# CSTR-Edinburgh/magphase

Measured on AMD Instinct MI355X. Metric: frames/sec analysis+synthesis @48kHz FFT=4096, higher is better.
Workload: dtype f32

## Files before the change

include/magphase_hip.h:

```cpp
#ifndef MAGPHASE_HIP_H
#define MAGPHASE_HIP_H

#include <stddef.h>
#include <stdint.h>

#ifdef __cplusplus
extern "C" {
#endif

#define MPX_ABI_VERSION 2

#define MPX_OK 0
#define MPX_ERR_ARG (-1)
#define MPX_ERR_HIP (-2)
#define MPX_ERR_HOST (-3)

int mpx_version(void);
const char* mpx_last_error(void);

size_t mpx_tables_bytes(int fft_len);
int mpx_tables_init(void* stream, int fft_len, void* tables);

int mpx_analysis_frames(void* stream, int fft_len, const void* tables, const float* sig,
                        const int64_t* frame_pos, const int32_t* frame_left, const int32_t* frame_right,
// ... 108 lines not shown
                                   const int32_t* frame_left, const int32_t* frame_right, const int64_t* scratch_off,
                                   int64_t n_frames, float* scratch, int64_t scratch_floats, float* grad_sig,
                                   int64_t total_smpls);

int mpx_analysis_lossless_const_rate_backward(void* stream, int fft_len, const void* tables, const float* mag,
                                              const float* real, const float* imag, int64_t ld, const float* grad_mag,
                                              const float* grad_real, const float* grad_imag, int64_t ld_grad,
                                              int64_t n_const_rows, const int32_t* ranges, const float* row_t,
                                              const int64_t* frame_pos, const int32_t* frame_left,
                                              const int32_t* frame_right, const int64_t* scratch_off, int64_t n_frames,
                                              float* scratch, int64_t scratch_floats, float* grad_sig,
                                              int64_t total_smpls);

int mpx_roundtrip_slot_weights(float* weights_host, int32_t n_slots);
int mpx_roundtrip_frame_terms(int fft_len, const int32_t* frame_left, const int32_t* frame_right, int64_t n_frames,
                              int32_t* terms_host);
int mpx_roundtrip_slot_costs(int32_t* coef_host, int32_t n_slots);
int mpx_roundtrip_lossless_ola(void* stream, int fft_len, const void* tables, const float* sig, const int64_t* frame_pos,
                               const int32_t* frame_left, const int32_t* frame_right, int64_t n_frames,
                               const mpx_ola_run* runs, int32_t n_runs, const int32_t* slot_off, const int32_t* slot_runs,
                               int32_t n_slots, const int32_t* pm_rel, float* out_mag, float* out_real, float* out_imag,
                               float* strips, float* pcm_out, int64_t ld);
#define MPX_RT_FULL_SUPPORT 1u
#define MPX_RT_STORE_ROWS 4u
#define MPX_RT_STORE_NT 8u
#define MPX_RT_INVERSE_TRANSFORM 32u
int mpx_roundtrip_store_map(int fft_len, int phase, int32_t* out);
int mpx_roundtrip_lossless_ola_flags(void* stream, int fft_len, const void* tables, const float* sig,
                                     const int64_t* frame_pos, const int32_t* frame_left, const int32_t* frame_right,
                                     int64_t n_frames, const mpx_ola_run* runs, int32_t n_runs, const int32_t* slot_off,
                                     const int32_t* slot_runs, int32_t n_slots, const int32_t* pm_rel, float* out_mag,
                                     float* out_real, float* out_imag, float* strips, float* pcm_out, int64_t ld,
                                     uint32_t flags);
int mpx_roundtrip_support_classes(int fft_len, const int32_t* frame_left, const int32_t* frame_right, int64_t n_frames,
                                  int32_t* class_host);
int mpx_roundtrip_frame_extents(int fft_len, const int32_t* frame_left, const int32_t* frame_right, int64_t n_frames,
                                uint32_t flags, int32_t* extents_host);

int mpx_griffin_lim_ola(void* stream, int fft_len, const void* tables, const float* sig_in, const int64_t* frame_pos,
                        const int32_t* frame_left, const int32_t* frame_right, int64_t n_frames, const float* target_mag,
                        const mpx_ola_run* runs, int32_t n_runs, const int32_t* slot_off, const int32_t* slot_runs,
                        int32_t n_slots, const int32_t* pm_rel, float* phase_out, float* strips, float* sig_out,
                        int64_t ld);

#define MPX_GL_FOLD_HALF 0
#define MPX_GL_FOLD_FULL 1
#define MPX_GL_FOLD_WORDS 2
int mpx_griffin_lim_fold(void* stream, int fft_len, int32_t form, const float* mag, const void* phase, int64_t ld_phase,
                         int64_t frame0, int64_t n_frames, float* out_mag, float* out_real, float* out_imag,
                         float* out_phase, int64_t ld);


int mpx_mel_unwarp(void* stream, int64_t n_frames, int32_t n_bins, const float* a_mag, int32_t k_mag,
                   const float* u_mag, float* out_mag, const float* a_real, const float* a_imag, int32_t k_phase,
                   const float* u_phase, float* out_real, float* out_imag,
                   int64_t ld );

int mpx_mel_unwarp_rows(void* stream, int64_t n_frames, int32_t n_bins, const float* a_mag, int32_t k_mag,
                        const float* u_mag, float* out_mag, const float* a_real, const float* a_imag, int32_t k_phase,
                        const float* u_phase, float* out_real, float* out_imag, int64_t ld, const int32_t* row0,
                        const int32_t* row1, const float* row_t, int64_t n_rows, const int32_t* tile_first,
                        const int32_t* voiced, int32_t n_phase_bins);

int64_t mpx_spec_ld(int32_t n_bins);

int mpx_noise_uniform(void* stream, int32_t n_utts, const uint64_t* seeds, const int64_t* offsets, int64_t max_len,
// ... 282 lines not shown
```

magphase_amd/_lib.py:

```python
import ctypes
import threading
import os

_HERE = os.path.dirname(os.path.abspath(__file__))
LIB_PATH = os.path.join(_HERE, "libmagphase_hip.so")

vp, i32, i64, sz, f64 = ctypes.c_void_p, ctypes.c_int32, ctypes.c_int64, ctypes.c_size_t, ctypes.c_double
u32 = ctypes.c_uint32

PROTOTYPES = {
    "mpx_version": (i32, []),
    "mpx_last_error": (ctypes.c_char_p, []),
    "mpx_tables_bytes": (sz, [i32]),
    "mpx_tables_init": (i32, [vp, i32, vp]),
    "mpx_feat_ld": (i64, [i32]),
    "mpx_analysis_frames": (i32, [vp, i32] + [vp] * 5 + [i64, vp, vp, vp, i64]),
    "mpx_tables_f64_bytes": (sz, [i32]),
    "mpx_tables_f64_init": (i32, [vp, i32, vp]),
    "mpx_analysis_frames_f64": (i32, [vp, i32] + [vp] * 5 + [i64, vp, vp, vp, i64, vp]),
    "mpx_analysis_frames_f64w": (i32, [vp, i32] + [vp] * 5 + [i64, vp, vp, vp, i64, vp, vp, i32]),
    "mpx_analysis_compressed_fused": (i32, [vp, i32] + [vp] * 5 + [i64, vp, i32, vp, vp, i32, i32, vp, i32, vp, vp,
                                       vp]),
    "mpx_analysis_compressed_fused_cr": (i32, [vp, i32] + [vp] * 5 + [i64, vp, i32, vp, vp, i32, i32] + [vp] * 4 +
                                          [i64] + [vp] * 4),
    "mpx_analysis_compressed_fused_cr_work_bytes": (i64, [i32, i64]),
    "mpx_analysis_compressed_fused_tiles": (i32, [i32, i32, ctypes.POINTER(i32), ctypes.POINTER(i32)]),
    "mpx_analysis_compressed_fused_waves": (i32, []),
    "mpx_analysis_compressed_fused_layout": (i32, []),
    "mpx_analysis_compressed_fused_blocks_per_cu": (i32, [i32, i32]),
    "mpx_synthesis_lossless_frames": (i32, [vp, i32] + [vp] * 4 + [i64, vp, i64]),
    "mpx_ola_gather": (i32, [vp, i32, vp, i32] + [vp] * 4 + [i64, vp]),
    "mpx_synth_ola_slots": (i32, []),
    "mpx_synth_ola_slot_weights": (i32, [vp, i32]),
    "mpx_ola_strip_floats": (i64, [i32]),
    "mpx_synthesis_lossless_ola": (i32, [vp, i32] + [vp] * 5 + [i32, vp, vp, i32, vp, vp, vp, i64]),
    "mpx_synthesis_lossless_ola_lerp": (i32, [vp, i32] + [vp] * 8 + [i32, vp, vp, i32, vp, vp, vp, i64]),
    "mpx_rows_lerp": (i32, [vp, i32, vp, vp, vp, i64, vp, vp, vp, i64, vp, vp, vp, i64]),
    "mpx_synthesis_lossless_backward": (i32, [vp, i32, vp, vp, i64, vp, vp, vp, i64, vp, vp, vp, i64] + [vp] * 6 + [i64]),
    "mpx_synthesis_compressed_backward": (i32, [vp, i32, vp, vp, i64, vp, vp, vp, i64, vp, vp, vp, i64] + [vp] * 12
                                          + [i32, vp, vp, vp, i64]),
    "mpx_synthesis_compressed_type2_backward": (i32, [vp, i32, vp, vp, i64, vp, vp, vp, i64, vp, vp, vp, i64] + [vp] * 12
                                                + [i32, vp, vp, vp, i64]),
    "mpx_rows_lerp_adjoint": (i32, [vp, i32, vp, vp, vp, i64, vp, vp, i64, vp, vp, vp, i64]),
    "mpx_analysis_lossless_backward": (i32, [vp, i32, vp, vp, vp, vp, i64, vp, vp, vp, i64, vp, vp, vp, vp, i64, vp, i64,
                                             vp, i64]),
    "mpx_analysis_lossless_const_rate_backward": (i32, [vp, i32, vp, vp, vp, vp, i64, vp, vp, vp, i64, i64, vp, vp, vp, vp,
                                                        vp, vp, i64, vp, i64, vp, i64]),
    "mpx_ola_fixup": (i32, [vp, i32, vp, i32, vp, vp]),
    "mpx_ola_fixup_width": (i32, [vp, i32, vp, i32, vp, vp, i32]),
    "mpx_roundtrip_lossless_ola": (i32, [vp, i32] + [vp] * 5 + [i64, vp, i32, vp, vp, i32] + [vp] * 6 + [i64]),
    "mpx_roundtrip_lossless_ola_flags": (i32, [vp, i32] + [vp] * 5 + [i64, vp, i32, vp, vp, i32] + [vp] * 6 + [i64, u32]),
    "mpx_roundtrip_support_classes": (i32, [i32, vp, vp, i64, vp]),
    "mpx_roundtrip_frame_extents": (i32, [i32, vp, vp, i64, u32, vp]),
    "mpx_roundtrip_store_map": (i32, [i32, i32, vp]),
    "mpx_roundtrip_slot_weights": (i32, [vp, i32]),
    "mpx_roundtrip_frame_terms": (i32, [i32, vp, vp, i64, vp]),
    "mpx_roundtrip_slot_costs": (i32, [vp, i32]),
    "mpx_griffin_lim_ola": (i32, [vp, i32] + [vp] * 5 + [i64, vp, vp, i32, vp, vp, i32] + [vp] * 4 + [i64]),
    "mpx_griffin_lim_fold": (i32, [vp, i32, i32, vp, vp, i64, i64, i64, vp, vp, vp, vp, i64]),
    "mpx_mel_unwarp": (i32, [vp, i64, i32, vp, i32] + [vp] * 4 + [i32, vp, vp, vp, i64]),
    "mpx_mel_unwarp_rows": (i32, [vp, i64, i32, vp, i32] + [vp] * 4 + [i32, vp, vp, vp, i64, vp, vp, vp, i64, vp, vp,
                             i32]),
    "mpx_spec_ld": (i64, [i32]),
    "mpx_noise_uniform": (i32, [vp, i32, vp, vp, i64, vp]),
    "mpx_noise_numpy_mt19937": (i32, [vp, vp, i32, i64] + [vp] * 5),
    "mpx_noise_numpy_mt19937_work_words": (i64, []),
    "mpx_host_mt19937_jump_poly": (i32, [i64, i32, vp]),
    "mpx_host_mt19937_jump_polys": (i32, [vp, i32, vp, i32]),
    "mpx_noise_stats": (i32, [vp, i32] + [vp] * 6 + [i64, vp]),
    "mpx_noise_spectra_floats": (i64, [i32, i64]),
    "mpx_noise_stats_spectra": (i32, [vp, i32] + [vp] * 6 + [i64, vp, vp]),
    "mpx_synth_comp_slots": (i32, []),
    "mpx_synth_comp_slot_weights": (i32, [vp, i32]),
    "mpx_synthesis_compressed_ola": (i32, [vp, i32] + [vp] * 21 + [i32, vp, vp, i32, vp, vp, i64, i32]),
    "mpx_synthesis_compressed_type2_ola": (i32, [vp, i32] + [vp] * 21 + [i32, vp, vp, i32, vp, vp, i64, i32]),
    "mpx_synthesis_compressed_ola_spectra": (i32, [vp, i32] + [vp] * 21 + [i32, vp, vp, i32, vp, vp, i64, i32, vp]),
    "mpx_host_const_to_var_scan": (i64, [vp, vp, i64, vp, vp]),
    "mpx_host_const_to_var_scan_cap": (i64, [vp, vp, i64, vp, vp, i64]),
    "mpx_host_plan_analysis": (i64, [i32] + [vp] * 12),
    "mpx_host_plan_analysis_batch": (i64, [i32] + [vp] * 8 + [i32] + [vp] * 9 + [i32, vp, vp, i64, vp, i32]),
    "mpx_host_plan_synthesis": (i64, [i32, vp, vp, f64, i32, i32, i32, i64] + [vp] * 17),
    "mpx_host_plan_synthesis_batch": (i64, [i32] + [vp] * 5 + [i32, i32, vp, vp, f64] + [i32] * 4 + [vp, f64, i32, vp,
                                       i64] + [vp] * 9 + [i64, vp, i32]),
    "mpx_host_plan_lossless_synthesis": (i64, [i32, vp, vp, vp, i32] + [vp] * 4),
# ... 25 lines not shown
    "mpx_post_filter": (i32, [vp, vp, i64, i32, vp, i32, i32, vp, vp]),
    "mpx_epoch_f0_track": (i32, [vp, vp, vp, i32, i32, vp, i64, vp, vp, vp, i64] + [i32] * 4 + [f64, vp, vp, vp]),
    "mpx_epoch_zff": (i32, [vp, vp, vp, i32, i64, vp, i32, vp, vp, vp, i32] + [vp] * 5),
    "mpx_pcm16": (i32, [vp, vp, i32, vp, i32, i64, f64, vp, vp]),
    "mpx_pcm16_to_f32": (i32, [vp, vp, i64, vp]),
    "mpx_hpf_block": (i32, []),
    "mpx_output_hpf": (i32, [vp] * 4 + [i32, i64] + [vp] * 7),
    "mpx_bw_probe": (i32, [vp, i32, vp, vp, i64]),
    "mpx_bw_probe_shapes": (i32, []),
    "mpx_rows_pack": (i32, [vp, vp, vp, i32, i32] + [vp, i32, i64, i64] * 3),
    "mpx_post_filter_merlin": (i32, [vp, vp, i64, i32] + [vp] * 4 + [i32, f64, vp, f64] + [vp] * 5),
    "mpx_post_filter_backward": (i32, [vp, vp, i64, i32, vp, vp, vp, i32, vp]),
    "mpx_post_filter_merlin_backward": (i32, [vp, vp, vp, i64, i32] + [vp] * 4 + [i32] + [vp] * 7),
    "mpx_mlpg_work_doubles": (i64, [i64, i32]),
    "mpx_mlpg_solve": (i32, [vp, vp, i32, i64, vp, i32, i64, vp, i32, i64, i32, i32, vp, i32, vp, i64, vp]),
    "mpx_mlpg_apply": (i32, [vp, vp, i32, i64, vp, i32, i64, vp, i32, i64, i32, i32, vp, vp, i64]),
    "mpx_mlpg_colsum_work_doubles": (i64, [i64, i64]),
    "mpx_mlpg_column_sums": (i32, [vp, vp, i64, i64, i64, vp, vp]),
    "mpx_mlpg_var_backward": (i32, [vp, vp, i64, vp, i64, vp, i32, i64, vp, i32, i64, vp, i32, i64, i32, i32, vp, vp, i64,
                                    vp, vp]),
    "mpx_mlpg_trajectory_nll": (i32, [vp, vp, i64, vp, i32, i64, vp, i32, i64, vp, i32, i64, i32, i32, vp, vp]),
    "mpx_mlpg_nll_work_doubles": (i64, [i64, i32]),
    "mpx_mlpg_trajectory_nll_backward": (i32, [vp, vp, i32, i64, vp, i32, i64, vp, i64, vp, i32, i64, vp, vp, i32, i64,
                                               i32, i32, vp, vp, i64, vp, i64, vp]),
    "mpx_cmp_voiced_neighbours": (i32, [vp, vp, i32, i64, vp, i32, i64, vp]),
    "mpx_cmp_compose": (i32, [vp, vp, i32, i64, vp, i32, i32, i32, f64, i32, vp, vp, i32, i64, i32, vp, vp, vp, vp, i32,
                              i64]),
    "mpx_cmp_compose_backward": (i32, [vp, vp, i64, vp, i32, i32, i32, vp, vp, i32, i64, i32, vp, vp, vp, i64]),
    "mpx_cmp_moments_work_doubles": (i64, [i64, i64]),
    "mpx_cmp_column_moments": (i32, [vp, vp, i32, i64, i64, i64, vp, vp]),
}
SYMBOLS = tuple(PROTOTYPES)
RT_STORE_FLAGS = {"rows": 4, "lines": 0, "lines_nt": 8}
RT_INVERSE_FLAGS = {"direct": 0, "transform": 32}
del vp, i32, i64, sz, f64

_lib = None


class MagphaseHipError(RuntimeError):
    pass


_load_lock = threading.Lock()


def load():
    global _lib
    if _lib is not None:
        return _lib
    with _load_lock:
        return _load_locked()


def _load_locked():
    global _lib
    if _lib is not None:
        return _lib
    import torch
    if not os.path.isfile(LIB_PATH):
        raise MagphaseHipError(
            "libmagphase_hip.so not found at %s -- build it with `python -m magphase_amd.build` "
            "(hipcc --offload-arch=gfx950). There is no CPU fallback." % LIB_PATH
        )
    lib = ctypes.CDLL(LIB_PATH)
    for name, (restype, argtypes) in PROTOTYPES.items():
# ... 11 lines not shown
```

magphase_amd/build.py:

```python
import hashlib
import os
import shutil
import subprocess
import sys
from concurrent.futures import ThreadPoolExecutor

HERE = os.path.dirname(os.path.abspath(__file__))
CSRC = os.path.join(HERE, "csrc")
UNITS = ["magphase_f64.hip", "magphase_warp.hip", "magphase_comp.hip", "magphase_hip.hip", "magphase_grad.hip",
         "magphase_grad_comp.hip", "magphase_grad_minphase.hip",
         "magphase_true_env.hip", "magphase_plan.cpp", "magphase_mtjump.cpp", "magphase_output.hip", "magphase_host.cpp",
         "magphase_epochs.hip", "magphase_noise.hip", "magphase_pack.hip", "magphase_probe.hip", "magphase_type2.hip",
         "magphase_merlin.hip", "magphase_mlpg.hip", "magphase_gl.hip", "magphase_cmp.hip"]
SRCS = [os.path.join(CSRC, u) for u in UNITS]
SRC = os.path.join(CSRC, "magphase_hip.hip")
HEADERS = [os.path.join(CSRC, "wave_fft.hpp"), os.path.join(CSRC, "wave_fft_f64.hpp"),
           os.path.join(CSRC, "mpx_common.hpp"), os.path.join(CSRC, "host_pool.hpp"),
           os.path.join(os.path.dirname(HERE), "include", "magphase_hip.h")]
PYHOST_SRC = os.path.join(CSRC, "magphase_pyhost.cpp")
PYHOST = os.path.join(HERE, "_mpx_pyhost.so")
DEPS = SRCS + HEADERS + [PYHOST_SRC]
LIB = os.path.join(HERE, "libmagphase_hip.so")
OBJ_DIR = os.path.join(HERE, "_obj")
CFLAGS = ["--offload-arch=gfx950", "-O3", "-std=c++17", "-fno-slp-vectorize", "-Wno-inline-asm", "-fPIC", "-pthread"]
FLAGS = CFLAGS + ["-shared"]
last_action = None


def hipcc_path():
    return shutil.which("hipcc") or "/opt/rocm/bin/hipcc"


def is_stale():
    if not os.path.isfile(LIB):
        return True
    t = os.path.getmtime(LIB)
    if any(os.path.getmtime(d) > t for d in DEPS):
        return True
    return _python_include() is not None and (not os.path.isfile(PYHOST) or os.path.getmtime(PYHOST) < t)


def _python_include():
    import sysconfig

    inc = sysconfig.get_paths().get("include")
    return inc if inc and os.path.isfile(os.path.join(inc, "Python.h")) else None


def build_pyhost(lib, verbose=True):
    inc = _python_include()
# ... 67 lines not shown
```

magphase_amd/csrc/magphase_comp.hip:

```cpp
#include <type_traits>

#include "mpx_common.hpp"

#ifndef MPX_COMP_PAIR_WAVES
#define MPX_COMP_PAIR_WAVES 12
#endif
#ifndef MPX_COMP_DIT
#define MPX_COMP_DIT 0
#endif
#ifndef MPX_COMP_CH
#define MPX_COMP_CH 16
#endif

namespace mpx {

template <int P, bool PRESTAGED, bool COMPACT, int W>
__device__ __forceinline__ void noise_window_gather(const FrameGeom& g, int wtype, float* xbuf, unsigned xbuf_byte, int lane,
                                                    float (&re)[P], float (&im)[P]) {
    constexpr int M = 64 * P, N = 2 * M, kTile = noise_tile_len(P, COMPACT);
    MPX_MARK("zero_init");
#pragma unroll
    for (int j = 0; j < P; ++j)
        if (j < W || j >= P - W) re[(COMPACT && MPX_COMP_DIT) ? brev(j, ilog2(P)) : j] = im[(COMPACT && MPX_COMP_DIT) ? brev(j, ilog2(P)) : j] = 0.0f;
    const int ntiles = MPX_NOISE_TILES(g.len, kTile);
// ... 1118 lines not shown
#endif
    while (cur.valid) {
        int lane;
        float wa_s, wa_c, ws_s, ws_c;
        pair_frame_lane<P>(w, lane, wa_s, wa_c, ws_s, ws_c);
        PairCursor nxt = cur;
        pair_cursor_advance(nxt, w.wi_end, w.half, runs, slot_runs);
        const int fi = cur.fi;
        bool narrow = false;
        if constexpr (kCls) narrow = MPX_RT_FORCE_NARROW || (frame_support_class(g.L, g.LR - g.L, N) == NW);

        float xr[P], xi[P];
        FrameGeom g_next = g;
        {
            float no_r[HP], no_i[HP], nm_r[HP], nm_i[HP], nh_r, nh_i;
            if constexpr (DIRECT) {
                auto on_gathered = [&](float (&re)[P], float (&im)[P], auto narrow_c) __attribute__((always_inline)) {
                    auto plain_sum = [](float o, float v, int) { return o + v; };
                    auto all_rows = [](int) { return true; };
                    pair_ordered_ola<P, true, NW, true>(w, cur, smem, runs, pm_rel, strips, pcm, re, im, lane, plain_sum,
                                                        all_rows, decltype(narrow_c)::value);
                };
                auto on_exchanged = [&]() __attribute__((always_inline)) {
                    if (nxt.valid) {
                        g_next = frame_geom(sig, fpos[nxt.fi], fleft[nxt.fi], fright[nxt.fi], N);
                        pair_stage_next<P>(w, g_next, lane);
                    }
                };
                pair_analysis_spectrum<P, NW>(w, g, lane, wa_c, wa_s, no_r, no_i, nm_r, nm_i, nh_r, nh_i, narrow,
                                              noise_fft_hook(on_gathered, on_exchanged));
            } else {
                pair_analysis_spectrum<P, NW>(w, g, lane, wa_c, wa_s, no_r, no_i, nm_r, nm_i, nh_r, nh_i, narrow);
            }
            MPX_MARK("features_stores_merge");
            auto feat = [](float x_r, float x_i, float& m, float& a, float& b) {
                const float s2 = x_r * x_r + x_i * x_i;
                const float r = __builtin_amdgcn_rsqf(fmaxf(s2, 1.0e-37f));
                m = s2 * r;
                a = x_r * r;
                b = x_i * r;
            };
            if constexpr (comp_compact<P>()) {
                const float4 pk = tw_half_pad<P>(w.tw, lane);
                ws_c = pk.x;
                ws_s = -pk.y;
            }
            const bool lane0 = (lane == 0);
            float* row_m = omag + (long long)fi * ld;
            float* row_r = oreal + (long long)fi * ld;
            float* row_i = oimag + (long long)fi * ld;
            int s_m = 0, s_r = 0, s_i = 0;
            if constexpr (ST != kStoreRows) {
                s_m = __builtin_amdgcn_readfirstlane(row_store_phase(row_m));
                s_r = __builtin_amdgcn_readfirstlane(row_store_phase(row_r));
                s_i = __builtin_amdgcn_readfirstlane(row_store_phase(row_i));
            }
            const bool pv_m = row_asc_prev(lane, s_m), pv_r = row_asc_prev(lane, s_r), pv_i = row_asc_prev(lane, s_i);
            const bool cu_m = row_mir_cur(lane, s_m), cu_r = row_mir_cur(lane, s_r), cu_i = row_mir_cur(lane, s_i);
            const int hoff = lane0 ? M - 64 : M - lane;
            float* mlo = row_m + (ST != kStoreRows ? 0 : lane);
            float* rlo = row_r + (ST != kStoreRows ? 0 : lane);
            float* ilo = row_i + (ST != kStoreRows ? 0 : lane);
            float* mhi = row_m + (ST != kStoreRows ? 0 : hoff);
            float* rhi = row_r + (ST != kStoreRows ? 0 : hoff);
            float* ihi = row_i + (ST != kStoreRows ? 0 : hoff);
            auto st_line = [](float* dst, float v) {
                if constexpr (ST == kStoreLinesNT) __builtin_nontemporal_store(v, dst);
                else *dst = v;
            };
            auto st_mask = [](float* dst, float v, unsigned long long mask) {
                unsigned long long saved;
                asm volatile("s_and_saveexec_b64 %0, %3\n\tglobal_store_dword %1, %2, off\n\ts_mov_b64 exec, %0"
                             : "=&s"(saved)
                             : "v"(dst), "v"(v), "s"(mask)
                             : "memory", "scc");
            };
            unsigned long long k_pv_m = 0, k_pv_r = 0, k_pv_i = 0, k_cu_m = 0, k_cu_r = 0, k_cu_i = 0;
            if constexpr (ST != kStoreRows) {
                k_pv_m = __builtin_amdgcn_ballot_w64(pv_m), k_cu_m = __builtin_amdgcn_ballot_w64(cu_m);
                k_pv_r = __builtin_amdgcn_ballot_w64(pv_r), k_cu_r = __builtin_amdgcn_ballot_w64(cu_r);
                k_pv_i = __builtin_amdgcn_ballot_w64(pv_i), k_cu_i = __builtin_amdgcn_ballot_w64(cu_i);
            }
            float zr[HP], zi[HP];
            float hm = 0.0f, ha = 0.0f, hb = 0.0f;
            float pm = 0.0f, pa = 0.0f, pb = 0.0f;
#pragma unroll
            for (int q = 0; q < HP; ++q) {
                float m, a, b, mq, aq, bq;
                feat(no_r[q], no_i[q], m, a, b);
                feat(nm_r[q], nm_i[q], mq, aq, bq);
                if constexpr (ST == kStoreRows) {
                    mlo[64 * q] = m;
                    rlo[64 * q] = a;
                    ilo[64 * q] = b;
                    if (q == 0) {
                        if (lane0) {
                            row_m[M] = mq;
                            row_r[M] = aq;
                            row_i[M] = bq;
                        }
                    } else {
                        mhi[-64 * (q - 1)] = lane0 ? mq : hm;
                        rhi[-64 * (q - 1)] = lane0 ? aq : ha;
                        ihi[-64 * (q - 1)] = lane0 ? bq : hb;
                    }
                } else if (q == 0) {
                    st_mask(mlo + row_asc_base(lane, false) + row_asc_off(0), m, ~k_pv_m);
                    st_mask(rlo + row_asc_base(lane, false) + row_asc_off(0), a, ~k_pv_r);
                    st_mask(ilo + row_asc_base(lane, false) + row_asc_off(0), b, ~k_pv_i);
                    if (cu_m || cu_r || cu_i) {
                        st_mask(mhi + row_mir_base(lane, true, M) + row_mir_off(0), mq, k_cu_m);
                        st_mask(rhi + row_mir_base(lane, true, M) + row_mir_off(0), aq, k_cu_r);
                        st_mask(ihi + row_mir_base(lane, true, M) + row_mir_off(0), bq, k_cu_i);
                    }
                } else {
                    st_line(mlo + row_asc_base(lane, pv_m) + row_asc_off(q), pv_m ? pm : m);
                    st_line(rlo + row_asc_base(lane, pv_r) + row_asc_off(q), pv_r ? pa : a);
                    st_line(ilo + row_asc_base(lane, pv_i) + row_asc_off(q), pv_i ? pb : b);
                    st_line(mhi + row_mir_base(lane, cu_m, M) + row_mir_off(q), cu_m ? mq : hm);
                    st_line(rhi + row_mir_base(lane, cu_r, M) + row_mir_off(q), cu_r ? aq : ha);
                    st_line(ihi + row_mir_base(lane, cu_i, M) + row_mir_off(q), cu_i ? bq : hb);
                }
                if constexpr (ST != kStoreRows) {
                    pm = m;
                    pa = a;
                    pb = b;
                }
                hm = mq;
                ha = aq;
                hb = bq;
                if constexpr (DIRECT) {
                    const float cq = cos2p<P>(q), sq = sin2p<P>(q);
                    const float wr = ws_c * cq - ws_s * sq, wi = ws_c * sq + ws_s * cq;
                    asm volatile("" ::"v"(wr), "v"(wi));
                } else {
                    const float x_r = no_r[q], p_r = nm_r[q];
                    float x_i = no_i[q], p_i = nm_i[q];
                    if (q == 0) {
                        x_i = lane0 ? 0.0f : x_i;
                        p_i = lane0 ? 0.0f : p_i;
                    }
                    merge_pair_step<P>(q, x_r, x_i, p_r, p_i, ws_c, ws_s, xr[q], xi[q], zr[q], zi[q]);
                }
            }
            float mH, aH, bH;
            feat(nh_r, nh_i, mH, aH, bH);
            if constexpr (ST == kStoreRows) {
                mhi[-64 * (HP - 1)] = lane0 ? mH : hm;
                rhi[-64 * (HP - 1)] = lane0 ? aH : ha;
                ihi[-64 * (HP - 1)] = lane0 ? bH : hb;
            } else {
                st_mask(mlo + row_asc_base(lane, true) + row_asc_off(HP), pm, k_pv_m);
                st_mask(rlo + row_asc_base(lane, true) + row_asc_off(HP), pa, k_pv_r);
                st_mask(ilo + row_asc_base(lane, true) + row_asc_off(HP), pb, k_pv_i);
                static_assert(row_mir_tail_live(0, true) && !row_mir_tail_live(1, true) && row_mir_tail_live(1, false),
                              "the mirror tail's lanes: lane 0 and those that do not store this step's mirror");
                st_mask(mhi + row_mir_base(lane, cu_m, M) + row_mir_off(HP), lane0 ? mH : hm, ~k_cu_m | 1ull);
                st_mask(rhi + row_mir_base(lane, cu_r, M) + row_mir_off(HP), lane0 ? aH : ha, ~k_cu_r | 1ull);
                st_mask(ihi + row_mir_base(lane, cu_i, M) + row_mir_off(HP), lane0 ? bH : hb, ~k_cu_i | 1ull);
            }
            if constexpr (!DIRECT) merge_handover<P>(zr, zi, 2.0f * nh_r, -2.0f * nh_i, xr, xi, lane);
        }
        if constexpr (DIRECT) {
            g = g_next;
        } else {
            pair_inverse_fft_front<P>(w, xr, xi, lane);
            if (nxt.valid) {
                g = frame_geom(sig, fpos[nxt.fi], fleft[nxt.fi], fright[nxt.fi], N);
                pair_stage_next<P>(w, g, lane);
            }
            if constexpr (kCls) pair_inverse_fft_back_class<P, NW>(xr, xi, narrow);
            else pair_inverse_fft_back<P>(xr, xi);
            constexpr float kScale = 0.5f / (float)M;
            auto plain_add = [](float o, float v, int) { return fmaf(v, kScale, o); };
            auto all_rows = [](int) { return true; };
            pair_ordered_ola<P, true, NW>(w, cur, smem, runs, pm_rel, strips, pcm, xr, xi, lane, plain_add, all_rows, narrow);
        }
        cur = nxt;
#ifdef MPX_PROBE_ENDTIME
        ++probe_frames;
#endif
    }
#ifdef MPX_PROBE_ENDTIME
    if (w.lane_id == 0) {
        const int pw = (blockIdx.x * kCompPairWaves + (int)(threadIdx.x >> 6)) % 8192;
        g_rt_endprobe[4 * pw + 0] = probe_t0;
        g_rt_endprobe[4 * pw + 1] = wall_clock64();
        g_rt_endprobe[4 * pw + 2] = (unsigned long long)probe_frames;
        g_rt_endprobe[4 * pw + 3] = clock64() - probe_c0;
    }
#endif
}

template <int P>
__global__ __launch_bounds__(kCompPairWaves * 64) void k_griffin_lim_pair(const float* __restrict__ sig,
                                                                         const long long* __restrict__ fpos,
                                                                         const int* __restrict__ fleft,
                                                                         const int* __restrict__ fright,
                                                                         const RunDesc* __restrict__ runs,
                                                                         const int* __restrict__ slot_off,
                                                                         const int* __restrict__ slot_runs, int nslots,
                                                                         const int* __restrict__ pm_rel,
                                                                         const float* __restrict__ tw_g,
                                                                         const float* __restrict__ tmag,
                                                                         float* __restrict__ phase_out,
                                                                         float* __restrict__ strips,
                                                                         float* __restrict__ pcm, long long ld) {
    constexpr int M = 64 * P, N = 2 * M, HP = P / 2;
    extern __shared__ __attribute__((aligned(16))) float smem[];
    PairWave w;
    if (!pair_wave_setup<P>(w, smem, tw_g, runs, slot_off, slot_runs, nslots)) return;
    PairCursor cur = w.cur;

    FrameGeom g = frame_geom(sig, fpos[cur.fi], fleft[cur.fi], fright[cur.fi], N);
    pair_stage_frame<P>(w, g, w.lane_id);

    while (cur.valid) {
        int lane;
        float wa_s, wa_c, ws_s, ws_c;
        pair_frame_lane<P>(w, lane, wa_s, wa_c, ws_s, ws_c);
        PairCursor nxt = cur;
        pair_cursor_advance(nxt, w.wi_end, w.half, runs, slot_runs);
        const int fi = cur.fi;

// ... 414 lines not shown
#define MPX_LAUNCH_RT(PP, CLS) MPX_LAUNCH_RT_K(PP, (k_roundtrip_pair<PP, CLS>))
#define MPX_LAUNCH_RT_K(PP, KERNEL)                                                                                    \
    do {                                                                                                             \
        auto KK = KERNEL;                                                                                            \
        if (int rc = set_lds(KK, lds_bytes_comp_pair<PP>())) return rc;                                              \
        hipLaunchKernelGGL(KK, pgrid, pblock, lds_bytes_comp_pair<PP>(), s, sig,                                     \
                           (const long long*)frame_pos, frame_left, frame_right, (const RunDesc*)runs, slot_off,     \
                           slot_runs, (int)n_slots, pm_rel, (const float*)tables, out_mag, out_real, out_imag, strips, \
                           pcm_out, (long long)ld);                                                                  \
    } while (0)
    if constexpr (kRtDirectBuilt) {
        if (P == 32 && !(flags & MPX_RT_INVERSE_TRANSFORM)) {
            if (flags & MPX_RT_FULL_SUPPORT) MPX_LAUNCH_RT_K(32, (k_roundtrip_pair<32, false, kStoreRows, true>));
            else if (flags & MPX_RT_STORE_ROWS) MPX_LAUNCH_RT_K(32, (k_roundtrip_pair<32, true, kStoreRows, true>));
            else if (flags & MPX_RT_STORE_NT) MPX_LAUNCH_RT_K(32, (k_roundtrip_pair<32, true, kStoreLinesNT, true>));
            else MPX_LAUNCH_RT_K(32, (k_roundtrip_pair<32, true, kStoreLines, true>));
            MPX_HIP_CHECK(hipGetLastError());
            return MPX_OK;
        }
    }
    if (P == 32 && !(flags & MPX_RT_FULL_SUPPORT)) {
        if (flags & MPX_RT_STORE_ROWS) MPX_LAUNCH_RT(32, true);
        else if (flags & MPX_RT_STORE_NT) MPX_LAUNCH_RT_K(32, (k_roundtrip_pair<32, true, kStoreLinesNT>));
        else MPX_LAUNCH_RT_K(32, (k_roundtrip_pair<32, true, kStoreLines>));
    } else if (P == 32) MPX_LAUNCH_RT(32, false);
    else if (P == 16) MPX_LAUNCH_RT(16, false);
    else MPX_LAUNCH_RT(8, false);
#undef MPX_LAUNCH_RT
#undef MPX_LAUNCH_RT_K
    MPX_HIP_CHECK(hipGetLastError());
    return MPX_OK;
}

int mpx_griffin_lim_ola(void* stream, int fft_len, const void* tables, const float* sig_in, const int64_t* frame_pos,
                        const int32_t* frame_left, const int32_t* frame_right, int64_t n_frames, const float* target_mag,
                        const mpx_ola_run* runs, int32_t n_runs, const int32_t* slot_off, const int32_t* slot_runs,
                        int32_t n_slots, const int32_t* pm_rel, float* phase_out, float* strips, float* sig_out,
                        int64_t ld) {
    const int P = p_of(fft_len);
    if (!P) return fail(MPX_ERR_ARG, "mpx_griffin_lim_ola: fft_len must be 1024, 2048 or 4096%s");
    if (n_frames < 0 || n_runs < 0 || n_slots < 0) return fail(MPX_ERR_ARG, "mpx_griffin_lim_ola: negative count%s");
    if (ld < fft_len / 2 + 1) return fail(MPX_ERR_ARG, "mpx_griffin_lim_ola: ld < fft_len/2 + 1%s");
    if (n_frames == 0 || n_runs == 0 || n_slots == 0) return MPX_OK;
    if (!tables || !sig_in || !frame_pos || !frame_left || !frame_right || !target_mag || !runs || !slot_off ||
        !slot_runs || !pm_rel || !strips || !sig_out)
        return fail(MPX_ERR_ARG, "mpx_griffin_lim_ola: null pointer%s");
    if (sig_in == sig_out) return fail(MPX_ERR_ARG, "mpx_griffin_lim_ola: sig_in and sig_out must be different buffers%s");
    hipStream_t s = (hipStream_t)stream;
    const dim3 pgrid((n_slots + kCompPairs - 1) / kCompPairs), pblock(kCompPairWaves * 64);
#define MPX_LAUNCH_GL(PP)                                                                                              \
    do {                                                                                                             \
        auto KK = k_griffin_lim_pair<PP>;                                                                            \
        if (int rc = set_lds(KK, lds_bytes_comp_pair<PP>())) return rc;                                              \
        hipLaunchKernelGGL(KK, pgrid, pblock, lds_bytes_comp_pair<PP>(), s, sig_in,                                  \
                           (const long long*)frame_pos, frame_left, frame_right, (const RunDesc*)runs, slot_off,     \
                           slot_runs, (int)n_slots, pm_rel, (const float*)tables, target_mag, phase_out, strips,     \
                           sig_out, (long long)ld);                                                                  \
    } while (0)
    if (P == 32) MPX_LAUNCH_GL(32);
    else if (P == 16) MPX_LAUNCH_GL(16);
    else MPX_LAUNCH_GL(8);
#undef MPX_LAUNCH_GL
    MPX_HIP_CHECK(hipGetLastError());
    return MPX_OK;
}

// ... 41 lines not shown
```

magphase_amd/engine.py:

```python
import ctypes
import os

import numpy as np

from . import _lib, hostmath as hm, hostplan


def _torch():
    import torch

    return torch


class HostTicket:

    def __init__(self, ring, slot, event, keep):
        self._ring, self._slot, self._event, self._keep = ring, slot, event, keep

    def wait(self):
        if self._event is not None:
            self._event.synchronize()
            self._event = self._keep = None

    def release(self):
# ... 30 lines not shown
        try:
            slot = self._freeq.get(timeout=timeout)
        except queue.Empty:
            return None, None
        try:
            with self._lock:
                buf = self._bufs[slot]
                if buf is None or buf.numel() < nbytes:
                    size = max([int(nbytes * 1.25), 1 << 20] + [b.numel() for b in self._bufs if b is not None])
                    self._bufs[slot] = buf = torch.empty(size, dtype=torch.uint8).pin_memory()
                    idle = []
                    while True:
                        try:
                            idle.append(self._freeq.get_nowait())
                        except queue.Empty:
                            break
                    try:
                        for k in idle:
                            if self._bufs[k] is None or self._bufs[k].numel() < size:
                                self._bufs[k] = torch.empty(size, dtype=torch.uint8).pin_memory()
                    finally:
                        for k in idle:
                            self._freeq.put(k)
        except BaseException:
            self._freeq.put(slot)
            raise
        return slot, buf

    def release(self, slot):
        self._freeq.put(slot)


class Engine:
    def __init__(self, device=None):
        torch = _torch()
        self.lib = _lib.load()
        if not torch.cuda.is_available():
            raise _lib.MagphaseHipError("magphase_amd needs a ROCm GPU (torch.cuda.is_available() is False); "
                                        "there is no CPU fallback")
        if device is None:
            device = torch.device("cuda", torch.cuda.current_device())
        self.device = torch.device(device)
        self._tables = {}

    def stream_ptr(self):
        return _torch().cuda.current_stream(self.device).cuda_stream

    def launch(self, name, *args):
        tensor = _torch().Tensor
        with _torch().cuda.device(self.device):
            rc = getattr(self.lib, name)(self.stream_ptr(), *[a.data_ptr() if isinstance(a, tensor) else a for a in args])
        if rc != 0:
            _lib.check(rc, name)

    def background(self, fn, *args):
        import concurrent.futures as cf

        if os.environ.get("MAGPHASE_HOST_THREAD", "1") == "0":
            f = cf.Future()
            try:
                f.set_result(fn(*args))
            except BaseException as exc:
                f.set_exception(exc)
            return f
        ex = getattr(self, "_helper", None)
        if ex is None:
# ... 863 lines not shown
    def tables_f64(self, fft_len):
        key = ("f64", fft_len)
        if key not in self._tables:
            torch = _torch()
            nbytes = self.lib.mpx_tables_f64_bytes(int(fft_len))
            if nbytes == 0:
                raise ValueError("fft_len %r not supported by the HIP path (1024, 2048 or 4096)" % (fft_len,))
            t = torch.empty(nbytes // 8, dtype=torch.float64, device=self.device)
            self.launch("mpx_tables_f64_init", int(fft_len), t)
            self._tables[key] = t
        return self._tables[key]

    def hann_table(self):
        t = getattr(self, "_hann_table", None)
        if t is None:
            t = self._hann_table = self.to_device(hm.hann_half_table(), np.float64)
        return t

    def hann_window_args(self):
        if os.environ.get("MAGPHASE_F64_WINDOW", "table") == "analytic":
            return None, 0
        return self.hann_table(), hm.HANN_TABLE_CAP

    def analysis_frames(self, fft_len, sig, pos, left, right, out=None, precise=False, rows_in_use=None):
        nfr = int(pos.numel())
        H = fft_len // 2 + 1
        if out is None:
            out = tuple(self.empty_feats(nfr, H) for _ in range(3))
        ld = self.feat_ld(*out)
        if precise:
            self.launch("mpx_analysis_frames_f64w", int(fft_len), self.tables_f64(fft_len), sig, pos, left, right, nfr,
                        out[0], out[1], out[2], ld, rows_in_use, *self.hann_window_args())
        else:
            self.launch("mpx_analysis_frames", int(fft_len), self.tables(fft_len), sig, pos, left, right, nfr,
                        out[0], out[1], out[2], ld)
        return out

    def synthesis_lossless_frames(self, fft_len, mag, real, imag, out=None):
        nfr = int(mag.shape[0])
        if out is None:
            out = self.empty((nfr, fft_len))
        self.launch("mpx_synthesis_lossless_frames", int(fft_len), self.tables(fft_len), mag, real, imag, nfr, out,
                    self.feat_ld(mag, real, imag))
        return out

    def ola_gather(self, fft_len, frames, utt_frame_off, pm_rel, out_start, out_off, max_out_len, total_out, out=None):
        if out is None:
            out = self.empty((int(total_out),))
        self.launch("mpx_ola_gather", int(fft_len), frames, int(out_start.numel()), utt_frame_off, pm_rel, out_start,
                    out_off, int(max_out_len), out)
        return out

    def synth_ola_slots(self):
        torch = _torch()
        with torch.cuda.device(self.device):
            n = int(self.lib.mpx_synth_ola_slots())
        cus = os.environ.get("MAGPHASE_SYN_CUS")
        return n if not cus else max(6, min(n, 6 * int(cus)))

    def synth_ola_slot_weights(self, comp=False):
        if os.environ.get("MAGPHASE_OLA_WEIGHTS", "1") == "0":
            return None
        key = ("rt_w" if comp == "roundtrip" else "comp_w") if comp else "ola_w"
        if key not in self._tables:
            n = self.synth_comp_slots() if comp else self.synth_ola_slots()
            w = np.zeros(n, dtype=np.float32)
            name = ("mpx_roundtrip_slot_weights" if comp == "roundtrip" else
                    "mpx_synth_comp_slot_weights") if comp else "mpx_synth_ola_slot_weights"
# ... 827 lines not shown
```

Before: 179.9 million.

## Add dedicated analysis kernel reusing roundtrip pair FFT front with line-aligned stores

Adds a new analysis-only kernel for FFT length 4096 that reuses the forward half of the roundtrip pair kernel: compact twiddle front, narrow support class, and prefetch of the next frame overlapped with the current frame's FFT. The feature/store block is moved into a shared include file so the roundtrip and new analysis kernels use the same code. Python now defaults to this path with non-temporal line-aligned stores instead of the classic analysis kernel, and the classic kernel stays available through a flag. This aims to cut analysis cost through better store coalescing and load overlap, but adds a separate code path whose correctness relies on the roundtrip kernel's pruning assumptions.

```diff
diff --git a/include/magphase_hip.h b/include/magphase_hip.h
--- a/include/magphase_hip.h
+++ b/include/magphase_hip.h
@@ -164,6 +164,10 @@
                                      const int32_t* slot_runs, int32_t n_slots, const int32_t* pm_rel, float* out_mag,
                                      float* out_real, float* out_imag, float* strips, float* pcm_out, int64_t ld,
                                      uint32_t flags);
+#define MPX_ANA_CLASSIC 64u
+int mpx_analysis_frames_flags(void* stream, int fft_len, const void* tables, const float* sig, const int64_t* frame_pos,
+                              const int32_t* frame_left, const int32_t* frame_right, int64_t n_frames, float* out_mag,
+                              float* out_real, float* out_imag, int64_t ld, uint32_t flags);
 int mpx_roundtrip_support_classes(int fft_len, const int32_t* frame_left, const int32_t* frame_right, int64_t n_frames,
                                   int32_t* class_host);
 int mpx_roundtrip_frame_extents(int fft_len, const int32_t* frame_left, const int32_t* frame_right, int64_t n_frames,
diff --git a/magphase_amd/_lib.py b/magphase_amd/_lib.py
--- a/magphase_amd/_lib.py
+++ b/magphase_amd/_lib.py
@@ -50,6 +50,7 @@
     "mpx_ola_fixup_width": (i32, [vp, i32, vp, i32, vp, vp, i32]),
     "mpx_roundtrip_lossless_ola": (i32, [vp, i32] + [vp] * 5 + [i64, vp, i32, vp, vp, i32] + [vp] * 6 + [i64]),
     "mpx_roundtrip_lossless_ola_flags": (i32, [vp, i32] + [vp] * 5 + [i64, vp, i32, vp, vp, i32] + [vp] * 6 + [i64, u32]),
+    "mpx_analysis_frames_flags": (i32, [vp, i32] + [vp] * 5 + [i64, vp, vp, vp, i64, u32]),
     "mpx_roundtrip_support_classes": (i32, [i32, vp, vp, i64, vp]),
     "mpx_roundtrip_frame_extents": (i32, [i32, vp, vp, i64, u32, vp]),
     "mpx_roundtrip_store_map": (i32, [i32, i32, vp]),
@@ -141,6 +142,7 @@
 }
 SYMBOLS = tuple(PROTOTYPES)
 RT_STORE_FLAGS = {"rows": 4, "lines": 0, "lines_nt": 8}
+ANALYSIS_FLAGS = dict(RT_STORE_FLAGS, classic=64)
 RT_INVERSE_FLAGS = {"direct": 0, "transform": 32}
 del vp, i32, i64, sz, f64
 
diff --git a/magphase_amd/build.py b/magphase_amd/build.py
--- a/magphase_amd/build.py
+++ b/magphase_amd/build.py
@@ -16,6 +16,7 @@
 SRC = os.path.join(CSRC, "magphase_hip.hip")
 HEADERS = [os.path.join(CSRC, "wave_fft.hpp"), os.path.join(CSRC, "wave_fft_f64.hpp"),
            os.path.join(CSRC, "mpx_common.hpp"), os.path.join(CSRC, "host_pool.hpp"),
+           os.path.join(CSRC, "pair_feature_rows.inc"),
            os.path.join(os.path.dirname(HERE), "include", "magphase_hip.h")]
 PYHOST_SRC = os.path.join(CSRC, "magphase_pyhost.cpp")
 PYHOST = os.path.join(HERE, "_mpx_pyhost.so")
diff --git a/magphase_amd/csrc/magphase_comp.hip b/magphase_amd/csrc/magphase_comp.hip
--- a/magphase_amd/csrc/magphase_comp.hip
+++ b/magphase_amd/csrc/magphase_comp.hip
@@ -1174,133 +1174,7 @@
             } else {
                 pair_analysis_spectrum<P, NW>(w, g, lane, wa_c, wa_s, no_r, no_i, nm_r, nm_i, nh_r, nh_i, narrow);
             }
-            MPX_MARK("features_stores_merge");
-            auto feat = [](float x_r, float x_i, float& m, float& a, float& b) {
-                const float s2 = x_r * x_r + x_i * x_i;
-                const float r = __builtin_amdgcn_rsqf(fmaxf(s2, 1.0e-37f));
-                m = s2 * r;
-                a = x_r * r;
-                b = x_i * r;
-            };
-            if constexpr (comp_compact<P>()) {
-                const float4 pk = tw_half_pad<P>(w.tw, lane);
-                ws_c = pk.x;
-                ws_s = -pk.y;
-            }
-            const bool lane0 = (lane == 0);
-            float* row_m = omag + (long long)fi * ld;
-            float* row_r = oreal + (long long)fi * ld;
-            float* row_i = oimag + (long long)fi * ld;
-            int s_m = 0, s_r = 0, s_i = 0;
-            if constexpr (ST != kStoreRows) {
-                s_m = __builtin_amdgcn_readfirstlane(row_store_phase(row_m));
-                s_r = __builtin_amdgcn_readfirstlane(row_store_phase(row_r));
-                s_i = __builtin_amdgcn_readfirstlane(row_store_phase(row_i));
-            }
-            const bool pv_m = row_asc_prev(lane, s_m), pv_r = row_asc_prev(lane, s_r), pv_i = row_asc_prev(lane, s_i);
-            const bool cu_m = row_mir_cur(lane, s_m), cu_r = row_mir_cur(lane, s_r), cu_i = row_mir_cur(lane, s_i);
-            const int hoff = lane0 ? M - 64 : M - lane;
-            float* mlo = row_m + (ST != kStoreRows ? 0 : lane);
-            float* rlo = row_r + (ST != kStoreRows ? 0 : lane);
-            float* ilo = row_i + (ST != kStoreRows ? 0 : lane);
-            float* mhi = row_m + (ST != kStoreRows ? 0 : hoff);
-            float* rhi = row_r + (ST != kStoreRows ? 0 : hoff);
-            float* ihi = row_i + (ST != kStoreRows ? 0 : hoff);
-            auto st_line = [](float* dst, float v) {
-                if constexpr (ST == kStoreLinesNT) __builtin_nontemporal_store(v, dst);
-                else *dst = v;
-            };
-            auto st_mask = [](float* dst, float v, unsigned long long mask) {
-                unsigned long long saved;
-                asm volatile("s_and_saveexec_b64 %0, %3\n\tglobal_store_dword %1, %2, off\n\ts_mov_b64 exec, %0"
-                             : "=&s"(saved)
-                             : "v"(dst), "v"(v), "s"(mask)
-                             : "memory", "scc");
-            };
-            unsigned long long k_pv_m = 0, k_pv_r = 0, k_pv_i = 0, k_cu_m = 0, k_cu_r = 0, k_cu_i = 0;
-            if constexpr (ST != kStoreRows) {
-                k_pv_m = __builtin_amdgcn_ballot_w64(pv_m), k_cu_m = __builtin_amdgcn_ballot_w64(cu_m);
-                k_pv_r = __builtin_amdgcn_ballot_w64(pv_r), k_cu_r = __builtin_amdgcn_ballot_w64(cu_r);
-                k_pv_i = __builtin_amdgcn_ballot_w64(pv_i), k_cu_i = __builtin_amdgcn_ballot_w64(cu_i);
-            }
-            float zr[HP], zi[HP];
-            float hm = 0.0f, ha = 0.0f, hb = 0.0f;
-            float pm = 0.0f, pa = 0.0f, pb = 0.0f;
-#pragma unroll
-            for (int q = 0; q < HP; ++q) {
-                float m, a, b, mq, aq, bq;
-                feat(no_r[q], no_i[q], m, a, b);
-                feat(nm_r[q], nm_i[q], mq, aq, bq);
-                if constexpr (ST == kStoreRows) {
-                    mlo[64 * q] = m;
-                    rlo[64 * q] = a;
-                    ilo[64 * q] = b;
-                    if (q == 0) {
-                        if (lane0) {
-                            row_m[M] = mq;
-                            row_r[M] = aq;
-                            row_i[M] = bq;
-                        }
-                    } else {
-                        mhi[-64 * (q - 1)] = lane0 ? mq : hm;
-                        rhi[-64 * (q - 1)] = lane0 ? aq : ha;
-                        ihi[-64 * (q - 1)] = lane0 ? bq : hb;
-                    }
-                } else if (q == 0) {
-                    st_mask(mlo + row_asc_base(lane, false) + row_asc_off(0), m, ~k_pv_m);
-                    st_mask(rlo + row_asc_base(lane, false) + row_asc_off(0), a, ~k_pv_r);
-                    st_mask(ilo + row_asc_base(lane, false) + row_asc_off(0), b, ~k_pv_i);
-                    if (cu_m || cu_r || cu_i) {
-                        st_mask(mhi + row_mir_base(lane, true, M) + row_mir_off(0), mq, k_cu_m);
-                        st_mask(rhi + row_mir_base(lane, true, M) + row_mir_off(0), aq, k_cu_r);
-                        st_mask(ihi + row_mir_base(lane, true, M) + row_mir_off(0), bq, k_cu_i);
-                    }
-                } else {
-                    st_line(mlo + row_asc_base(lane, pv_m) + row_asc_off(q), pv_m ? pm : m);
-                    st_line(rlo + row_asc_base(lane, pv_r) + row_asc_off(q), pv_r ? pa : a);
-                    st_line(ilo + row_asc_base(lane, pv_i) + row_asc_off(q), pv_i ? pb : b);
-                    st_line(mhi + row_mir_base(lane, cu_m, M) + row_mir_off(q), cu_m ? mq : hm);
-                    st_line(rhi + row_mir_base(lane, cu_r, M) + row_mir_off(q), cu_r ? aq : ha);
-                    st_line(ihi + row_mir_base(lane, cu_i, M) + row_mir_off(q), cu_i ? bq : hb);
-                }
-                if constexpr (ST != kStoreRows) {
-                    pm = m;
-                    pa = a;
-                    pb = b;
-                }
-                hm = mq;
-                ha = aq;
-                hb = bq;
-                if constexpr (DIRECT) {
-                    const float cq = cos2p<P>(q), sq = sin2p<P>(q);
-                    const float wr = ws_c * cq - ws_s * sq, wi = ws_c * sq + ws_s * cq;
-                    asm volatile("" ::"v"(wr), "v"(wi));
-                } else {
-                    const float x_r = no_r[q], p_r = nm_r[q];
-                    float x_i = no_i[q], p_i = nm_i[q];
-                    if (q == 0) {
-                        x_i = lane0 ? 0.0f : x_i;
-                        p_i = lane0 ? 0.0f : p_i;
-                    }
-                    merge_pair_step<P>(q, x_r, x_i, p_r, p_i, ws_c, ws_s, xr[q], xi[q], zr[q], zi[q]);
-                }
-            }
-            float mH, aH, bH;
-            feat(nh_r, nh_i, mH, aH, bH);
-            if constexpr (ST == kStoreRows) {
-                mhi[-64 * (HP - 1)] = lane0 ? mH : hm;
-                rhi[-64 * (HP - 1)] = lane0 ? aH : ha;
-                ihi[-64 * (HP - 1)] = lane0 ? bH : hb;
-            } else {
-                st_mask(mlo + row_asc_base(lane, true) + row_asc_off(HP), pm, k_pv_m);
-                st_mask(rlo + row_asc_base(lane, true) + row_asc_off(HP), pa, k_pv_r);
-                st_mask(ilo + row_asc_base(lane, true) + row_asc_off(HP), pb, k_pv_i);
-                static_assert(row_mir_tail_live(0, true) && !row_mir_tail_live(1, true) && row_mir_tail_live(1, false),
-                              "the mirror tail's lanes: lane 0 and those that do not store this step's mirror");
-                st_mask(mhi + row_mir_base(lane, cu_m, M) + row_mir_off(HP), lane0 ? mH : hm, ~k_cu_m | 1ull);
-                st_mask(rhi + row_mir_base(lane, cu_r, M) + row_mir_off(HP), lane0 ? aH : ha, ~k_cu_r | 1ull);
-                st_mask(ihi + row_mir_base(lane, cu_i, M) + row_mir_off(HP), lane0 ? bH : hb, ~k_cu_i | 1ull);
-            }
+#include "pair_feature_rows.inc"
             if constexpr (!DIRECT) merge_handover<P>(zr, zi, 2.0f * nh_r, -2.0f * nh_i, xr, xi, lane);
         }
         if constexpr (DIRECT) {
@@ -1332,6 +1206,79 @@
         g_rt_endprobe[4 * pw + 3] = clock64() - probe_c0;
     }
 #endif
+}
+
+#ifndef MPX_ANA_LINES_QUEUE
+#define MPX_ANA_LINES_QUEUE 0
+#endif
+template <int P>
+constexpr size_t lds_bytes_ana_lines() {
+    return sizeof(float) * (size_t)(comp_tw_floats<P>() + kCompPairWaves * comp_xbuf_floats<P>() + 4);
+}
+template <int P, int ST>
+__global__ __launch_bounds__(kCompPairWaves * 64) void k_analysis_lines(const float* __restrict__ sig,
+                                                                       const long long* __restrict__ fpos,
+                                                                       const int* __restrict__ fleft,
+                                                                       const int* __restrict__ fright, long long nframes,
+                                                                       const float* __restrict__ tw_g,
+                                                                       float* __restrict__ omag, float* __restrict__ oreal,
+                                                                       float* __restrict__ oimag, long long ld) {
+    constexpr int M = 64 * P, N = 2 * M, HP = P / 2, NW = kSupportNarrow;
+    constexpr bool DIRECT = (P == 32);
+    static_assert(P == 32 && comp_compact<P>() && roundtrip_prunes<P>(true) && kRtDirectBuilt,
+                  "the forward half of k_roundtrip_pair<32, true, ST, true>: compact transform front, narrow class");
+    extern __shared__ __attribute__((aligned(16))) float smem[];
+    const int wave = rfl((int)(threadIdx.x >> 6));
+    PairWave w = {};
+    w.tw = smem;
+    w.lane_id = threadIdx.x & 63;
+    w.xbuf = smem + comp_tw_floats<P>() + wave * comp_xbuf_floats<P>();
+    w.xbuf_byte = 4u * (unsigned)(comp_tw_floats<P>() + wave * comp_xbuf_floats<P>());
+    unsigned* queue = reinterpret_cast<unsigned*>(smem + comp_tw_floats<P>() + kCompPairWaves * comp_xbuf_floats<P>());
+    if (threadIdx.x == 0) *queue = 0u;
+    pair_kernel_prologue<P, true, MPX_COMP_DIT != 0>(w.tw, tw_g, nullptr, 0, nullptr, 0, kCompPairWaves * 64);
+
+#if MPX_ANA_LINES_QUEUE
+    long long fb, fe;
+    block_frame_range(nframes, fb, fe);
+    long long fi = queue_pull(queue, fb);
+#else
+    const long long fe = nframes, fstep = (long long)gridDim.x * kCompPairWaves;
+    long long fi = (long long)blockIdx.x * kCompPairWaves + wave;
+#endif
+    if (fi >= fe) return;
+    FrameGeom g = frame_geom(sig, fpos[fi], fleft[fi], fright[fi], N);
+    pair_stage_frame<P>(w, g, w.lane_id);
+
+    while (true) {
+        int lane;
+        float wa_s, wa_c, ws_s, ws_c;
+        pair_frame_lane<P>(w, lane, wa_s, wa_c, ws_s, ws_c);
+#if MPX_ANA_LINES_QUEUE
+        const long long fn = queue_pull(queue, fb);
+#else
+        const long long fn = fi + fstep;
+#endif
+        const bool narrow = MPX_RT_FORCE_NARROW || (frame_support_class(g.L, g.LR - g.L, N) == NW);
+        FrameGeom g_next = g;
+        {
+            float no_r[HP], no_i[HP], nm_r[HP], nm_i[HP], nh_r, nh_i;
+            float xr[P], xi[P];
+            auto on_gathered = [](float (&)[P], float (&)[P], auto) __attribute__((always_inline)) {};
+            auto on_exchanged = [&]() __attribute__((always_inline)) {
+                if (fn < fe) {
+                    g_next = frame_geom(sig, fpos[fn], fleft[fn], fright[fn], N);
+                    pair_stage_next<P>(w, g_next, lane);
+                }
+            };
+            pair_analysis_spectrum<P, NW>(w, g, lane, wa_c, wa_s, no_r, no_i, nm_r, nm_i, nh_r, nh_i, narrow,
+                                          noise_fft_hook(on_gathered, on_exchanged));
+#include "pair_feature_rows.inc"
+        }
+        if (fn >= fe) break;
+        g = g_next;
+        fi = fn;
+    }
 }
 
 template <int P>
@@ -1812,6 +1759,39 @@
     return MPX_OK;
 }
 
+int mpx_analysis_frames_flags(void* stream, int fft_len, const void* tables, const float* sig, const int64_t* frame_pos,
+                              const int32_t* frame_left, const int32_t* frame_right, int64_t n_frames, float* out_mag,
+                              float* out_real, float* out_imag, int64_t ld, uint32_t flags) {
+    if (flags & ~(MPX_ANA_CLASSIC | MPX_RT_STORE_ROWS | MPX_RT_STORE_NT))
+        return fail(MPX_ERR_ARG, "mpx_analysis_frames_flags: unknown flag%s");
+    if ((flags & MPX_RT_STORE_ROWS) && (flags & MPX_RT_STORE_NT))
+        return fail(MPX_ERR_ARG, "mpx_analysis_frames_flags: MPX_RT_STORE_NT needs the line-aligned stores%s");
+    if (fft_len != 4096 || (flags & MPX_ANA_CLASSIC))
+        return mpx_analysis_frames(stream, fft_len, tables, sig, frame_pos, frame_left, frame_right, n_frames, out_mag,
+                                   out_real, out_imag, ld);
+    if (n_frames < 0) return fail(MPX_ERR_ARG, "mpx_analysis_frames_flags: negative n_frames%s");
+    if (ld < fft_len / 2 + 1) return fail(MPX_ERR_ARG, "mpx_analysis_frames_flags: ld < fft_len/2 + 1%s");
+    if (n_frames == 0) return MPX_OK;
+    if (!tables || !sig || !frame_pos || !frame_left || !frame_right || !out_mag || !out_real || !out_imag)
+        return fail(MPX_ERR_ARG, "mpx_analysis_frames_flags: null pointer%s");
+    const dim3 grid(grid_for(n_frames, kCompPairWaves)), block(kCompPairWaves * 64);
+    hipStream_t s = (hipStream_t)stream;
+#define MPX_LAUNCH_ANA(ST)                                                                                              \
+    do {                                                                                                               \
+        auto KK = k_analysis_lines<32, ST>;                                                                            \
+        if (int rc = set_lds(KK, lds_bytes_ana_lines<32>())) return rc;                                                \
+        hipLaunchKernelGGL(KK, grid, block, lds_bytes_ana_lines<32>(), s, sig, (const long long*)frame_pos, frame_left, \
+                           frame_right, (long long)n_frames, (const float*)tables, out_mag, out_real, out_imag,        \
+                           (long long)ld);                                                                             \
+    } while (0)
+    if (flags & MPX_RT_STORE_ROWS) MPX_LAUNCH_ANA(kStoreRows);
+    else if (flags & MPX_RT_STORE_NT) MPX_LAUNCH_ANA(kStoreLinesNT);
+    else MPX_LAUNCH_ANA(kStoreLines);
+#undef MPX_LAUNCH_ANA
+    MPX_HIP_CHECK(hipGetLastError());
+    return MPX_OK;
+}
+
 int mpx_griffin_lim_ola(void* stream, int fft_len, const void* tables, const float* sig_in, const int64_t* frame_pos,
                         const int32_t* frame_left, const int32_t* frame_right, int64_t n_frames, const float* target_mag,
                         const mpx_ola_run* runs, int32_t n_runs, const int32_t* slot_off, const int32_t* slot_runs,
diff --git a/magphase_amd/csrc/pair_feature_rows.inc b/magphase_amd/csrc/pair_feature_rows.inc
--- /dev/null
+++ b/magphase_amd/csrc/pair_feature_rows.inc
@@ -0,0 +1,127 @@
+            MPX_MARK("features_stores_merge");
+            auto feat = [](float x_r, float x_i, float& m, float& a, float& b) {
+                const float s2 = x_r * x_r + x_i * x_i;
+                const float r = __builtin_amdgcn_rsqf(fmaxf(s2, 1.0e-37f));
+                m = s2 * r;
+                a = x_r * r;
+                b = x_i * r;
+            };
+            if constexpr (comp_compact<P>()) {
+                const float4 pk = tw_half_pad<P>(w.tw, lane);
+                ws_c = pk.x;
+                ws_s = -pk.y;
+            }
+            const bool lane0 = (lane == 0);
+            float* row_m = omag + (long long)fi * ld;
+            float* row_r = oreal + (long long)fi * ld;
+            float* row_i = oimag + (long long)fi * ld;
+            int s_m = 0, s_r = 0, s_i = 0;
+            if constexpr (ST != kStoreRows) {
+                s_m = __builtin_amdgcn_readfirstlane(row_store_phase(row_m));
+                s_r = __builtin_amdgcn_readfirstlane(row_store_phase(row_r));
+                s_i = __builtin_amdgcn_readfirstlane(row_store_phase(row_i));
+            }
+            const bool pv_m = row_asc_prev(lane, s_m), pv_r = row_asc_prev(lane, s_r), pv_i = row_asc_prev(lane, s_i);
+            const bool cu_m = row_mir_cur(lane, s_m), cu_r = row_mir_cur(lane, s_r), cu_i = row_mir_cur(lane, s_i);
+            const int hoff = lane0 ? M - 64 : M - lane;
+            float* mlo = row_m + (ST != kStoreRows ? 0 : lane);
+            float* rlo = row_r + (ST != kStoreRows ? 0 : lane);
+            float* ilo = row_i + (ST != kStoreRows ? 0 : lane);
+            float* mhi = row_m + (ST != kStoreRows ? 0 : hoff);
+            float* rhi = row_r + (ST != kStoreRows ? 0 : hoff);
+            float* ihi = row_i + (ST != kStoreRows ? 0 : hoff);
+            auto st_line = [](float* dst, float v) {
+                if constexpr (ST == kStoreLinesNT) __builtin_nontemporal_store(v, dst);
+                else *dst = v;
+            };
+            auto st_mask = [](float* dst, float v, unsigned long long mask) {
+                unsigned long long saved;
+                asm volatile("s_and_saveexec_b64 %0, %3\n\tglobal_store_dword %1, %2, off\n\ts_mov_b64 exec, %0"
+                             : "=&s"(saved)
+                             : "v"(dst), "v"(v), "s"(mask)
+                             : "memory", "scc");
+            };
+            unsigned long long k_pv_m = 0, k_pv_r = 0, k_pv_i = 0, k_cu_m = 0, k_cu_r = 0, k_cu_i = 0;
+            if constexpr (ST != kStoreRows) {
+                k_pv_m = __builtin_amdgcn_ballot_w64(pv_m), k_cu_m = __builtin_amdgcn_ballot_w64(cu_m);
+                k_pv_r = __builtin_amdgcn_ballot_w64(pv_r), k_cu_r = __builtin_amdgcn_ballot_w64(cu_r);
+                k_pv_i = __builtin_amdgcn_ballot_w64(pv_i), k_cu_i = __builtin_amdgcn_ballot_w64(cu_i);
+            }
+            float zr[HP], zi[HP];
+            float hm = 0.0f, ha = 0.0f, hb = 0.0f;
+            float pm = 0.0f, pa = 0.0f, pb = 0.0f;
+#pragma unroll
+            for (int q = 0; q < HP; ++q) {
+                float m, a, b, mq, aq, bq;
+                feat(no_r[q], no_i[q], m, a, b);
+                feat(nm_r[q], nm_i[q], mq, aq, bq);
+                if constexpr (ST == kStoreRows) {
+                    mlo[64 * q] = m;
+                    rlo[64 * q] = a;
+                    ilo[64 * q] = b;
+                    if (q == 0) {
+                        if (lane0) {
+                            row_m[M] = mq;
+                            row_r[M] = aq;
+                            row_i[M] = bq;
+                        }
+                    } else {
+                        mhi[-64 * (q - 1)] = lane0 ? mq : hm;
+                        rhi[-64 * (q - 1)] = lane0 ? aq : ha;
+                        ihi[-64 * (q - 1)] = lane0 ? bq : hb;
+                    }
+                } else if (q == 0) {
+                    st_mask(mlo + row_asc_base(lane, false) + row_asc_off(0), m, ~k_pv_m);
+                    st_mask(rlo + row_asc_base(lane, false) + row_asc_off(0), a, ~k_pv_r);
+                    st_mask(ilo + row_asc_base(lane, false) + row_asc_off(0), b, ~k_pv_i);
+                    if (cu_m || cu_r || cu_i) {
+                        st_mask(mhi + row_mir_base(lane, true, M) + row_mir_off(0), mq, k_cu_m);
+                        st_mask(rhi + row_mir_base(lane, true, M) + row_mir_off(0), aq, k_cu_r);
+                        st_mask(ihi + row_mir_base(lane, true, M) + row_mir_off(0), bq, k_cu_i);
+                    }
+                } else {
+                    st_line(mlo + row_asc_base(lane, pv_m) + row_asc_off(q), pv_m ? pm : m);
+                    st_line(rlo + row_asc_base(lane, pv_r) + row_asc_off(q), pv_r ? pa : a);
+                    st_line(ilo + row_asc_base(lane, pv_i) + row_asc_off(q), pv_i ? pb : b);
+                    st_line(mhi + row_mir_base(lane, cu_m, M) + row_mir_off(q), cu_m ? mq : hm);
+                    st_line(rhi + row_mir_base(lane, cu_r, M) + row_mir_off(q), cu_r ? aq : ha);
+                    st_line(ihi + row_mir_base(lane, cu_i, M) + row_mir_off(q), cu_i ? bq : hb);
+                }
+                if constexpr (ST != kStoreRows) {
+                    pm = m;
+                    pa = a;
+                    pb = b;
+                }
+                hm = mq;
+                ha = aq;
+                hb = bq;
+                if constexpr (DIRECT) {
+                    const float cq = cos2p<P>(q), sq = sin2p<P>(q);
+                    const float wr = ws_c * cq - ws_s * sq, wi = ws_c * sq + ws_s * cq;
+                    asm volatile("" ::"v"(wr), "v"(wi));
+                } else {
+                    const float x_r = no_r[q], p_r = nm_r[q];
+                    float x_i = no_i[q], p_i = nm_i[q];
+                    if (q == 0) {
+                        x_i = lane0 ? 0.0f : x_i;
+                        p_i = lane0 ? 0.0f : p_i;
+                    }
+                    merge_pair_step<P>(q, x_r, x_i, p_r, p_i, ws_c, ws_s, xr[q], xi[q], zr[q], zi[q]);
+                }
+            }
+            float mH, aH, bH;
+            feat(nh_r, nh_i, mH, aH, bH);
+            if constexpr (ST == kStoreRows) {
+                mhi[-64 * (HP - 1)] = lane0 ? mH : hm;
+                rhi[-64 * (HP - 1)] = lane0 ? aH : ha;
+                ihi[-64 * (HP - 1)] = lane0 ? bH : hb;
+            } else {
+                st_mask(mlo + row_asc_base(lane, true) + row_asc_off(HP), pm, k_pv_m);
+                st_mask(rlo + row_asc_base(lane, true) + row_asc_off(HP), pa, k_pv_r);
+                st_mask(ilo + row_asc_base(lane, true) + row_asc_off(HP), pb, k_pv_i);
+                static_assert(row_mir_tail_live(0, true) && !row_mir_tail_live(1, true) && row_mir_tail_live(1, false),
+                              "the mirror tail's lanes: lane 0 and those that do not store this step's mirror");
+                st_mask(mhi + row_mir_base(lane, cu_m, M) + row_mir_off(HP), lane0 ? mH : hm, ~k_cu_m | 1ull);
+                st_mask(rhi + row_mir_base(lane, cu_r, M) + row_mir_off(HP), lane0 ? aH : ha, ~k_cu_r | 1ull);
+                st_mask(ihi + row_mir_base(lane, cu_i, M) + row_mir_off(HP), lane0 ? bH : hb, ~k_cu_i | 1ull);
+            }
diff --git a/magphase_amd/engine.py b/magphase_amd/engine.py
--- a/magphase_amd/engine.py
+++ b/magphase_amd/engine.py
@@ -86,6 +86,8 @@
 
 
 class Engine:
+    DEFAULT_ANALYSIS = "lines_nt"
+
     def __init__(self, device=None):
         torch = _torch()
         self.lib = _lib.load()
@@ -1015,8 +1017,11 @@
             self.launch("mpx_analysis_frames_f64w", int(fft_len), self.tables_f64(fft_len), sig, pos, left, right, nfr,
                         out[0], out[1], out[2], ld, rows_in_use, *self.hann_window_args())
         else:
-            self.launch("mpx_analysis_frames", int(fft_len), self.tables(fft_len), sig, pos, left, right, nfr,
-                        out[0], out[1], out[2], ld)
+            form = os.environ.get("MAGPHASE_ANALYSIS", "") or self.DEFAULT_ANALYSIS
+            if form not in _lib.ANALYSIS_FLAGS:
+                raise ValueError("MAGPHASE_ANALYSIS must be classic, rows, lines or lines_nt, not %r" % form)
+            self.launch("mpx_analysis_frames_flags", int(fft_len), self.tables(fft_len), sig, pos, left, right, nfr,
+                        out[0], out[1], out[2], ld, _lib.ANALYSIS_FLAGS[form])
         return out
 
     def synthesis_lossless_frames(self, fft_len, mag, real, imag, out=None):
```

New measurement: 172.3 million. -4.2%, worse.
